# jianfch/stable-ts

Measured on AMD Instinct MI355X. Metric: real-time factor (audio-sec/wall-sec) large-v3 word_timestamps=True, higher is better.
Workload: dtype f16; 1 GPU; large-v3 (random-init, weight recipe BENCH_WEIGHTS = the parity-pinned recipe of tests/test_gpu_f16_depth.py), 10 min synthetic 16 kHz audio per GPU, word_timestamps=True, beam_size=5, 112 decode steps/window, window-parallel batch 20, default regrouping inside the timed pass; mode=transcribe, windows_per_gpu=20, segments=125, words=1670, parallelism=dp1 (windows sharded, no data-path collective)

## Files before the change

### include/swx.h

```cpp
#ifndef SWX_H
#define SWX_H
#include <stdint.h>
#include <stddef.h>

#ifdef __cplusplus
extern "C" {
#endif

#define SWX_F32 0
#define SWX_F16 1

#define SWX_N_SAMPLES 480000
#define SWX_N_FRAMES 3000
#define SWX_N_FFT 400
#define SWX_HOP 160

typedef struct swx_dims {
    int32_t n_mels, n_audio_ctx, n_audio_state, n_audio_head, n_audio_layer;
    int32_t n_vocab, n_text_ctx, n_text_state, n_text_head, n_text_layer;
} swx_dims;

typedef struct swx_model swx_model;

const char *swx_strerror(int code);
// ... 99 lines not shown
int swx_pcm_edit(const float *d_clean, float *d_probe, int64_t stride, int n_rows, const int32_t *d_ops,
                 const int32_t *d_row_start, int n_ops, void *stream);

typedef struct swx_flac_info {
    int32_t sample_rate, channels, bits_per_sample, min_block, max_block;
    int64_t total_samples;
    uint8_t md5[16];
} swx_flac_info;
int swx_flac_probe(const uint8_t *h_data, size_t n_bytes, swx_flac_info *info);
int64_t swx_flac_decode(const uint8_t *h_data, size_t n_bytes, int32_t *h_out, int64_t capacity_frames, swx_flac_info *info);

size_t swx_dtw_workspace_bytes(int W, int ld_n, int ld_m);
int swx_dtw(const float *d_x, int W, int ld_n, int ld_m, const int32_t *d_N, const int32_t *d_M,
            int32_t *d_text_idx, int32_t *d_time_idx, int32_t *d_len, void *d_trace_ws, void *stream);

int swx_prof_enable(int on);
int swx_debug_flags(int flags);
int swx_prof_collect(double *out, int n_classes);
int swx_graph_stats(const swx_model *m, int64_t *out);

int swx_test_gemm(int dtype, const void *d_a, int64_t lda, const void *d_w, const float *d_bias, const void *d_res,
                  void *d_c, int64_t ldc, int M, int N, int K, int epilogue, int force_kernel, void *stream);
int swx_test_gemm_plan(int M, int N, int K, int epilogue, int force_kernel, int flags);
int swx_test_dec_gemm(const void *d_a, int64_t lda, const void *d_w, const float *d_gamma, const float *d_beta,
                      const float *d_bias, void *d_c, int64_t ldc, void *d_x, void *d_kcache, void *d_vcache,
                      const int32_t *d_pos0, int n_ctx, int d, int M, int N, int K, int epilogue, void *d_scratch,
                      size_t scratch_bytes, void *stream);
int swx_test_layernorm(int dtype, const void *d_x, const float *d_g, const float *d_b, void *d_y, int rows, int d,
                       void *stream);
int swx_test_attention(int dtype, const void *d_q, int64_t ldq, const void *d_k, const void *d_v, int64_t ldkv,
                       void *d_o, int64_t ldo, int B, int H, int nq, int nk, int force_kernel, int vt_kp, void *stream);

int swx_test_self_attn_step(const void *d_q, void *d_kcache, void *d_vcache, const int32_t *d_anc, const int32_t *d_pos0,
                            int R, int H, int n_ctx, int d, int variant, void *d_o, void *stream);

int swx_test_self_attn_multi(const void *d_q, void *d_kcache, void *d_vcache, int R, int H, int n_new, int n_ctx, int d, int mq,
                             void *d_o, void *stream);

int swx_test_self_attn_general(int dtype, const void *d_qkv, int64_t ldqkv, void *d_kcache, void *d_vcache, const int32_t *d_anc,
                               const int32_t *d_pos0, int R, int H, int n_new, int n_ctx, int d, int row_mul, int skip_append,
                               int pos0_all_zero, void *d_o, void *stream);
int swx_test_kcache_index(int k_chunked, int n_ctx, int d, int pos, int h, int chunk);
int swx_test_kcache_relayout(const void *h_src, void *h_dst, int64_t rows, int n_ctx, int d, int elem_bytes, int to_chunked);
int swx_test_dec_gemm_kl(const void *d_a, int64_t lda, const void *d_w, const float *d_gamma, const float *d_beta,
                         const float *d_bias, void *d_c, int64_t ldc, void *d_x, void *d_kcache, void *d_vcache,
                         const int32_t *d_pos0, int n_ctx, int d, int M, int N, int K, int epilogue, int rps, int k_chunked,
// ... 30 lines not shown
```

### stable_ts_amd/_lib.py

```python
import ctypes
import os
from ctypes import POINTER, Structure, c_char_p, c_float, c_int, c_int32, c_int64, c_size_t, c_uint64, c_void_p

_HERE = os.path.dirname(os.path.abspath(__file__))
LIB_PATH = os.path.join(_HERE, "libswx.so")

SWX_F32 = 0
SWX_F16 = 1


class SwxError(RuntimeError):
    pass


class swx_dims(Structure):
    _fields_ = [(n, c_int32) for n in ("n_mels", "n_audio_ctx", "n_audio_state", "n_audio_head", "n_audio_layer",
                                       "n_vocab", "n_text_ctx", "n_text_state", "n_text_head", "n_text_layer")]


class swx_flac_info(Structure):
    _fields_ = [("sample_rate", c_int32), ("channels", c_int32), ("bits_per_sample", c_int32), ("min_block", c_int32),
                ("max_block", c_int32), ("total_samples", c_int64), ("md5", ctypes.c_uint8 * 16)]


# ... 54 lines not shown
                                       c_void_p, c_void_p, c_void_p, c_void_p]),
    "swx_test_next_token_reduce": (c_int, [c_void_p, c_int64, c_int, c_int, c_void_p, c_int, c_void_p, c_void_p, c_void_p,
                                           c_void_p]),
    "swx_detect_language": (c_int, [c_void_p, c_void_p, c_int, c_int, c_void_p, c_int, c_void_p, c_void_p, c_void_p]),
    "swx_align_weights_scratch_bytes":(c_size_t, [c_int, c_int, c_int]),
    "swx_align_weights": (c_int, [c_void_p, c_int, c_int, c_int, c_int, POINTER(c_int32), c_float, c_int, c_void_p,
                                  c_void_p, c_size_t, c_void_p]),
    "swx_median_filter": (c_int, [c_void_p, c_int64, c_int, c_int, c_void_p, c_void_p]),
    "swx_loudness_probe": (c_int, [c_void_p, c_int64, c_void_p, c_void_p, c_int, c_int, c_void_p, c_void_p, c_size_t, c_void_p]),
    "swx_loudness_probe_scratch_bytes": (c_size_t, [c_int]),
    "swx_pcm_edit": (c_int, [c_void_p, c_void_p, c_int64, c_int, c_void_p, c_void_p, c_int, c_void_p]),
    "swx_flac_probe": (c_int, [c_void_p, c_size_t, POINTER(swx_flac_info)]),
    "swx_flac_decode": (c_int64, [c_void_p, c_size_t, c_void_p, c_int64, POINTER(swx_flac_info)]),
    "swx_dtw_workspace_bytes": (c_size_t, [c_int, c_int, c_int]),
    "swx_dtw": (c_int, [c_void_p, c_int, c_int, c_int, c_void_p, c_void_p, c_void_p, c_void_p, c_void_p, c_void_p,
                        c_void_p]),
    "swx_prof_enable": (c_int, [c_int]),
    "swx_debug_flags": (c_int, [c_int]),
    "swx_prof_collect": (c_int, [POINTER(ctypes.c_double), c_int]),
    "swx_graph_stats": (c_int, [c_void_p, POINTER(c_int64)]),
    "swx_test_gemm": (c_int, [c_int, c_void_p, c_int64, c_void_p, c_void_p, c_void_p, c_void_p, c_int64, c_int, c_int,
                              c_int, c_int, c_int, c_void_p]),
    "swx_test_gemm_plan": (c_int, [c_int, c_int, c_int, c_int, c_int, c_int]),
    "swx_test_dec_gemm": (c_int, [c_void_p, c_int64, c_void_p, c_void_p, c_void_p, c_void_p, c_void_p, c_int64, c_void_p,
                                  c_void_p, c_void_p, c_void_p, c_int, c_int, c_int, c_int, c_int, c_int, c_void_p, c_size_t,
                                  c_void_p]),
    "swx_test_self_attn_step": (c_int, [c_void_p, c_void_p, c_void_p, c_void_p, c_void_p, c_int, c_int, c_int, c_int, c_int, c_void_p,
                                        c_void_p]),
    "swx_test_self_attn_multi": (c_int, [c_void_p, c_void_p, c_void_p, c_int, c_int, c_int, c_int, c_int, c_int, c_void_p, c_void_p]),
    "swx_test_self_attn_general": (c_int, [c_int, c_void_p, c_int64, c_void_p, c_void_p, c_void_p, c_void_p, c_int, c_int, c_int, c_int,
                                           c_int, c_int, c_int, c_int, c_void_p, c_void_p]),
    "swx_test_kcache_index": (c_int, [c_int] * 6),
    "swx_test_kcache_relayout": (c_int, [c_void_p, c_void_p, c_int64, c_int, c_int, c_int, c_int]),
    "swx_test_dec_gemm_kl": (c_int, [c_void_p, c_int64, c_void_p, c_void_p, c_void_p, c_void_p, c_void_p, c_int64, c_void_p,
                                     c_void_p, c_void_p, c_void_p, c_int, c_int, c_int, c_int, c_int, c_int, c_int, c_int, c_void_p,
                                     c_size_t, c_void_p]),
    "swx_test_self_attn_step_kl": (c_int, [c_void_p, c_void_p, c_void_p, c_void_p, c_void_p, c_int, c_int, c_int, c_int, c_int, c_int,
                                           c_void_p, c_void_p]),
    "swx_test_self_attn_multi_kl": (c_int, [c_void_p, c_void_p, c_void_p, c_int, c_int, c_int, c_int, c_int, c_int, c_int, c_void_p,
                                            c_void_p]),
    "swx_test_self_attn_general_kl": (c_int, [c_int, c_void_p, c_int64, c_void_p, c_void_p, c_void_p, c_void_p, c_int, c_int, c_int,
                                              c_int, c_int, c_int, c_int, c_int, c_int, c_int, c_void_p, c_void_p]),
    "swx_test_self_attn_plan": (c_int, [c_int] * 12),
    "swx_test_dec_plan": (c_int, [c_int, c_int, c_int, c_int, c_int]),
    "swx_test_gelu_pair": (c_int, [c_void_p, c_void_p]),
    "swx_test_decode_script_ws_bytes": (c_size_t, [POINTER(swx_decode_cfg), c_int, c_int]),
# ... 44 lines not shown
```

### stable_ts_amd/csrc/swx_gemm.hip

```cpp
#include <cstdlib>
#include <type_traits>
#include <array>
#include <vector>
#include <cstdio>
#include "swx_common.h"
#include "swx_kernels.h"

namespace {

template <typename T>
__device__ __forceinline__ void epilogue_store(const GemmArgs &g, int row, int col, float v)
{
    if (row >= g.M || col >= g.N) return;
    if (g.epi & EPI_BIAS) v += g.bias[col];
    if (g.epi & EPI_GELU) v = gelu_erf(v);
    if (g.epi & EPI_RESF32MOD) v += g.Rf[(size_t)(row % g.res_mod) * g.N + col];
    if (g.epi & EPI_RES) v += to_f32<T>(((const T *)g.R)[(size_t)row * g.ldr + col]);
    if (g.epi & EPI_STORE_VT) {
        const int w = row / g.vt_s, sidx = row - w * g.vt_s;
        ((T *)g.C)[(size_t)w * g.vt_bs + (size_t)col * g.vt_kp + sidx] = from_f32<T>(v);
    } else if (g.epi & EPI_CBATCH) {
        const int w = row / g.vt_s, sidx = row - w * g.vt_s;
        ((T *)g.C)[(size_t)w * g.vt_bs + (size_t)sidx * g.ldc + col] = from_f32<T>(v);
    } else if (g.epi & EPI_OUT_F32) ((float *)g.C)[(size_t)row * g.ldc + col] = v;
// ... 967 lines not shown
    if (K % 32 != 0) return -4;
    const bool skinny_ok = M <= 128 && K % 128 == 0 && K / 128 <= 10 && N <= 16384;
    if (force_kernel == 2) return skinny_ok ? SWX_GEMM_SKINNY : -4;
    if (skinny_ok && force_kernel != 1 && force_kernel < 7) return SWX_GEMM_SKINNY;
    const bool glds_ok = K % 64 == 0 && ptr16;
    if (force_kernel >= 7 && !glds_ok) return -4;
    if (force_kernel == 1 || !glds_ok) return SWX_GEMM_TILED_REG;
    const int64_t t128 = (int64_t)cdiv(N, BN) * cdiv(M, BM);
    const bool narrow = force_kernel == 8 || (force_kernel != 9 && N % 64 == 0 && t128 < 224);
    const bool big_ok = !(epi & ~(EPI_BIAS | EPI_GELU | EPI_RES)) && ldc % 8 == 0 && (!(epi & EPI_RES) || ldr % 8 == 0);
    if (force_kernel == 12) return big_ok && K >= 128 ? SWX_GEMM_BIG : -4;
    const int64_t t256 = (int64_t)cdiv(M, BG) * cdiv(N, BG);
    const double fill = (double)t256 / (double)(((t256 + 255) / 256) * 256);
    if (force_kernel == 0 && big_ok && t256 >= 200 && K >= 512 && (fill >= 0.9 || (fill >= 0.75 && K >= 2560)) &&
        !(flags & SWX_FLAG_NO_BIG_TILE))
        return SWX_GEMM_BIG;
    const bool ring_ok = K >= 128;
    if (force_kernel == 10 || force_kernel == 11) return !ring_ok ? -4 : force_kernel == 10 ? SWX_GEMM_RING64 : SWX_GEMM_RING128;
    if (force_kernel == 0 && ring_ok && M > 256 && (narrow || t128 <= 256) && !(flags & SWX_FLAG_NO_RING))
        return narrow ? SWX_GEMM_RING64 : SWX_GEMM_RING128;
    return narrow ? SWX_GEMM_GLDS64 : SWX_GEMM_GLDS128;
}

int swx_gemm(int dtype, const GemmArgs &g, int force_kernel, hipStream_t s)
{
    if (g.M <= 0 || g.N <= 0) return 0;
    if (dtype == SWX_F16) {
        if (g.lda % 8 != 0 || g.ldw % 8 != 0) return -4;
        const bool ptr16 = (uintptr_t)g.A % 16 == 0 && (uintptr_t)g.W % 16 == 0;
        const bool cr16 = (uintptr_t)g.C % 16 == 0 && (!(g.epi & EPI_RES) || (uintptr_t)g.R % 16 == 0);
        const int plan = swx_gemm_plan_f16(g.M, g.N, g.K, g.epi, cr16 ? g.ldc : 1, cr16 ? g.ldr : 1, ptr16, force_kernel, swx_flags());
        if (plan < 0) return plan;
        if (plan == SWX_GEMM_SKINNY) {
            SwxProfScope prof(PC_GEMM_SKINNY, 2.0 * ((double)g.N * g.K + (double)g.M * g.K) + (double)g.M * g.N * ((g.epi & EPI_OUT_F32) ? 4 : 2), s);
            dim3 grid(cdiv(g.N, 16));
            const int mt = cdiv(g.M, 16);
            switch (mt) {
                case 1: hipLaunchKernelGGL(gemm_f16_skinny<1>, grid, dim3(256), 0, s, g); break;
                case 2: hipLaunchKernelGGL(gemm_f16_skinny<2>, grid, dim3(256), 0, s, g); break;
                case 3: hipLaunchKernelGGL(gemm_f16_skinny<3>, grid, dim3(256), 0, s, g); break;
                case 4: hipLaunchKernelGGL(gemm_f16_skinny<4>, grid, dim3(256), 0, s, g); break;
                case 5: hipLaunchKernelGGL(gemm_f16_skinny<5>, grid, dim3(256), 0, s, g); break;
                case 6: hipLaunchKernelGGL(gemm_f16_skinny<6>, grid, dim3(256), 0, s, g); break;
                case 7: hipLaunchKernelGGL(gemm_f16_skinny<7>, grid, dim3(256), 0, s, g); break;
                default: hipLaunchKernelGGL(gemm_f16_skinny<8>, grid, dim3(256), 0, s, g); break;
            }
        } else {
            SwxProfScope prof(PC_GEMM_TILED, 2.0 * (double)g.M * g.N * g.K, s);
            const dim3 grid(cdiv(g.N, BN), cdiv(g.M, BM));
            switch (plan) {
                case SWX_GEMM_BIG: {
                    GemmArgs gb = g;
                    gb.tile_order = (swx_flags() & SWX_FLAG_BIG8_GROUPED) ? 1 : 0;
                    hipLaunchKernelGGL(gemm_f16_big8, dim3(cdiv(g.N, BG), cdiv(g.M, BG)), dim3(512), 2 * B8_BUF, s, gb); break;
// ... 25 lines not shown
```

### stable_ts_amd/csrc/swx_kernels.h

```cpp
#pragma once
#include <hip/hip_runtime.h>
#include <stdint.h>
#include "../../include/swx.h"

#define EPI_BIAS 1
#define EPI_GELU 2
#define EPI_RES 4
#define EPI_OUT_F32 8
#define EPI_RESF32MOD 16
#define EPI_CBATCH 64
#define EPI_STORE_VT 32
#define EPI_KV 128

#define EPI_QKV_VT 256

struct GemmArgs {
    const void *A; int64_t lda;
    const void *W; int64_t ldw;
    const float *bias;
    const void *R; int64_t ldr;
    const float *Rf; int res_mod;
    void *C; int64_t ldc;
    void *C2;
    void *P; int64_t p_bs;
    int p_nkpad, p_vcol0;
    int M, N, K;
    int epi;
    int vt_s, vt_kp; int64_t vt_bs;
    int vt_zero_pad;
    int tile_order;
};
int swx_gemm(int dtype, const GemmArgs &g, int force_kernel, hipStream_t s);
enum { SWX_GEMM_TILED_REG = 0, SWX_GEMM_SKINNY = 1, SWX_GEMM_GLDS128 = 2, SWX_GEMM_GLDS64 = 3, SWX_GEMM_RING64 = 4, SWX_GEMM_RING128 = 5,
       SWX_GEMM_BIG = 6 };
int swx_gemm_plan_f16(int M, int N, int K, int epi, int64_t ldc, int64_t ldr, bool ptr16, int force_kernel, int flags);

#define SWX_FLAG_NO_FAST_STEP 1
#define SWX_FLAG_NO_PACKED_XKV 2048
#define SWX_FLAG_SELECT_MEM 8192
#define SWX_FLAG_NO_GRAPH 16384
#define SWX_FLAG_NO_PREFETCH 32768
#define SWX_FLAG_NO_RING 65536
#define SWX_FLAG_SCORE_TILED 262144
#define SWX_FLAG_NO_TALL 524288
#define SWX_FLAG_NO_FUSED_XQ 1048576
#define SWX_FLAG_TICKET 2097152
#define SWX_FLAG_BIG8_GROUPED 4194304
#define SWX_FLAG_XKV_TWO_LAUNCHES 8388608
#define SWX_FLAG_LOUDNESS_ONE_WG 16777216
#define SWX_FLAG_XATTN_R5 33554432
#define SWX_FLAG_FLASH_PIPELINED 67108864
#define SWX_FLAG_SELFATTN_WG5 134217728
#define SWX_FLAG_QKV_SEPARATE_VT 268435456
#define SWX_FLAG_SELFATTN_NO_DEEP 4
#define SWX_FLAG_DEC_NO_W1 16
#define SWX_FLAG_TALL_NO_W8 32
#define SWX_FLAG_SELFATTN_NO_MQ 256
#define SWX_FLAG_FLASH_NO_QB1 64
#define SWX_FLAG_XKV_PACK_SEPARATE 128
#define SWX_FLAG_DEC_W1_FULL_TILE 256
#define SWX_FLAG_XQ_FULL_TILE 512
#define SWX_FLAG_KCACHE_CHUNKED 2
#define SWX_FLAG_NO_BIG_TILE 131072
#define SWX_DEFAULT_FLAGS 0
int swx_flags();

struct KLayout { int sp, sh, sc; };
__host__ __device__ inline KLayout swx_klayout(int chunked, int n_ctx, int d)
{
    return chunked ? KLayout{8, 64 * n_ctx, 8 * n_ctx} : KLayout{d, 64, 8};
}
__host__ __device__ inline int swx_kidx(const KLayout &L, int pos, int h, int chunk) { return h * L.sh + chunk * L.sc + pos * L.sp; }

#define DEC_LN 1
#define DEC_GELU 2
#define DEC_RES 4
#define DEC_QKV 8
#define DEC_SLAB 16
#define DEC_TICKET 32
struct DecPrefetch {
    const void *base;
    int lines;
};
DecPrefetch swx_dec_prefetch_of(const void *packed_w, int M, int N, int K, int epi);

struct DecGemmArgs {
    const _Float16 *A; int64_t lda;
    const _Float16 *W; int64_t ldw;
// ... 124 lines not shown
```

### stable_ts_amd/csrc/swx_runtime.hip

```cpp
#include <algorithm>
#include <map>
#include <memory>
#include <string>
#include <vector>
#include <cmath>
#include <cstring>
#include <cstdio>
#include <cstdlib>
#include "swx_common.h"
#include "swx_kernels.h"
#include "swx_decode.h"

namespace {

enum SlotKind { SK_MAT = 0, SK_VEC = 1, SK_CONV = 2 };

struct Slot {
    size_t off = 0;
    int kind = SK_VEC;
    int64_t rows = 0, cols = 0;
    int64_t dst_ld = 0;
    bool loaded = false;
};

// ... 36 lines not shown
        size_t tokens0, tokens1, anc0, anc1, pos0, win_begin, sum_lp, sum_lp_next, row_done, win_done, win_done_prev, n_done;
        size_t fin_tokens, fin_score, fin_len, fin_count, cand_lp, cand_tok, logits, hid2;
        size_t kcache, vcache, sk, sv, cap, mean, sd, suppress, slabs, heads, win_uid;
        size_t total;
        int64_t rows_big, logits_rows;
        size_t slab_bytes;
    } L;

    template <typename P> P *A(size_t off) const { return (P *)(arena + off); }
    template <typename P> P *Wp(size_t off) const { return (P *)(ws + off); }

    struct StepGraph { std::vector<uint64_t> key; hipGraph_t graph = nullptr; hipGraphExec_t exec = nullptr; uint64_t used = 0; };
    std::vector<StepGraph> graphs;
    uint64_t graph_clock = 0;
    std::vector<int32_t> ragged_hv;
    hipStream_t cap_stream = nullptr;
    bool graphs_off = false;
    int graph_failures = 0;
    int64_t n_captures = 0, n_replays = 0, n_eager_units = 0;
    void drop_graphs() {
        for (auto &g : graphs) { if (g.exec) (void)hipGraphExecDestroy(g.exec); if (g.graph) (void)hipGraphDestroy(g.graph); }
        graphs.clear();
    }
    ~swx_model() { drop_graphs(); if (cap_stream) (void)hipStreamDestroy(cap_stream); }
};

namespace {

constexpr int FIN_CAP = 32;
constexpr int MAX_GROUP = 16;
constexpr int MAX_SUPPRESS = 4096;
constexpr int SMALL_I32 = 8192;

size_t add_slot(swx_model *m, size_t &cur, const std::string &name, int kind, int64_t rows, int64_t cols, int64_t dst_ld,
                size_t bytes, size_t base_off = (size_t)-1, size_t sub_off = 0)
{
    Slot s;
    s.kind = kind; s.rows = rows; s.cols = cols; s.dst_ld = dst_ld;
    if (base_off == (size_t)-1) { s.off = cur; cur = align_up(cur + bytes); }
    else s.off = base_off + sub_off;
    m->slots[name] = s;
    return s.off;
}

void build_layout(swx_model *m)
{
    const swx_dims &D = m->dims;
// ... 177 lines not shown

hipEvent_t prof_event()
{
    if (g_pool_next == g_pool.size()) {
        hipEvent_t e;
        if (hipEventCreate(&e) != hipSuccess) return nullptr;
        g_pool.push_back(e);
    }
    return g_pool[g_pool_next++];
}

#define SWX_TRY(expr) do { int _r = (expr); if (_r < 0) return _r; } while (0)

GemmArgs gemm_args(const void *A, int64_t lda, const void *W, int64_t ldw, const float *bias, void *C, int64_t ldc,
                   int M, int N, int K, int epi)
{
    GemmArgs g{};
    g.A = A; g.lda = lda; g.W = W; g.ldw = ldw; g.bias = bias; g.C = C; g.ldc = ldc; g.M = M; g.N = N; g.K = K; g.epi = epi;
    g.R = nullptr; g.ldr = 0; g.Rf = nullptr; g.res_mod = 1;
    return g;
}

int gemm_residual(swx_model *m, const void *A, int64_t lda, size_t w_off, size_t b_off, void *X, int64_t ldx, int M, int N,
                  int K, hipStream_t s)
{
    GemmArgs g = gemm_args(A, lda, m->arena + w_off, K, m->A<float>(b_off), X, ldx, M, N, K, EPI_BIAS | EPI_RES);
    g.R = X; g.ldr = ldx;
    return swx_gemm(m->dtype, g, 0, s);
}

inline int64_t xkv_plain_elems(const swx_dims &D)
{
    return (int64_t)D.n_audio_ctx * D.n_text_state + (int64_t)D.n_text_state * SWX_VT_KP;
}
inline int64_t xkv_packed_elems(const swx_dims &D)
{
    return (int64_t)D.n_text_head * swx_xkv_packed_elems_per_head(D.n_audio_ctx);
}
inline int64_t xkv_chunk_elems(const swx_model *m)
{
    return xkv_plain_elems(m->dims) + (m->dtype == SWX_F16 ? xkv_packed_elems(m->dims) : 0);
}

struct FwdCfg {
    int W;
    int rpw;
    int row_mul;
    int n_new;
    const int32_t *tokens; int64_t ld_tok;
    int xkv_W;
    const int32_t *pos0;
    unsigned char *kcache, *vcache;
// ... 464 lines not shown
    __syncthreads();
    mx = fmaxf(fmaxf(red[0], red[1]), fmaxf(red[2], red[3]));
    __syncthreads();
    float sum = 0.f;
    for (int j = tid; j < n_lang; j += 256) {
        const float x = lg[j];
        if (x == mx) atomicMin(&best_j, j);
        const float p = expf(x - mx);
        lg[j] = p;
        sum += p;
    }
    sum = wave_sum(sum);
    if (lane == 0) red[wave] = sum;
    __syncthreads();
    sum = (red[0] + red[1]) + (red[2] + red[3]);
    for (int j = tid; j < n_lang; j += 256) probs[(size_t)w * n_lang + j] = lg[j] / sum;
    if (tid == 0) best[w] = best_j < n_lang ? lang_tokens[best_j] : -1;
}

}

bool swx_prof_on() { return g_prof_enabled; }
int swx_flags() { return g_debug_flags; }
void swx_prof_begin(int cls, double work, hipStream_t s)
{
    ProfRec r{cls, work, prof_event(), prof_event()};
    if (!r.a || !r.b) return;
    (void)hipEventRecord(r.a, s);
    g_prof.push_back(r);
}
void swx_prof_end(hipStream_t s)
{
    if (!g_prof.empty()) (void)hipEventRecord(g_prof.back().b, s);
}

__global__ __launch_bounds__(64) void lane_xor_check_kernel(const uint32_t *__restrict__ in, uint32_t *__restrict__ out)
{
    const int lane = threadIdx.x;
    const uint32_t x = in[blockIdx.x * 64 + lane];
    uint32_t *o = out + (size_t)blockIdx.x * 13 * 64 + lane;
    o[0 * 64] = lane_xor_u32<32>(x, lane); o[1 * 64] = lane_xor_u32<16>(x, lane); o[2 * 64] = lane_xor_u32<8>(x, lane);
    o[3 * 64] = lane_xor_u32<4>(x, lane);  o[4 * 64] = lane_xor_u32<2>(x, lane);  o[5 * 64] = lane_xor_u32<1>(x, lane);
    o[6 * 64] = (uint32_t)__shfl_xor((int)x, 32, 64); o[7 * 64] = (uint32_t)__shfl_xor((int)x, 16, 64);
    o[8 * 64] = (uint32_t)__shfl_xor((int)x, 8, 64);  o[9 * 64] = (uint32_t)__shfl_xor((int)x, 4, 64);
    o[10 * 64] = (uint32_t)__shfl_xor((int)x, 2, 64); o[11 * 64] = (uint32_t)__shfl_xor((int)x, 1, 64);
    double v = (double)__uint_as_float(x);
// ... 282 lines not shown
    std::vector<int32_t> lens((size_t)B * 2);
    for (int b = 0; b < B; ++b) {
        if (n_total[b] <= 200 || n_total[b] / 160 > 3008 || n_valid[b] < 0 || n_valid[b] > n_total[b] ||
            n_valid[b] > 480000)
            return -2;
        lens[2 * b] = n_valid[b];
        lens[2 * b + 1] = n_total[b];
    }
    hipStream_t s = S(stream);
    int32_t *d_lens = m->Wp<int32_t>(m->L.h1);
    hipError_t e = hipMemcpyAsync(d_lens, lens.data(), lens.size() * 4, hipMemcpyHostToDevice, s);
    if (e == hipSuccess) e = hipStreamSynchronize(s);
    if (e != hipSuccess) return -100 - (int)e;
    return swx_mel_ragged_launch(d_pcm, d_lens, B, m->A<float>(m->o_hann), m->A<double2>(m->o_twiddle),
                                 m->A<float>(m->o_filters), m->dims.n_mels, d_mel, m->Wp<unsigned>(m->L.gmax), group, s);
}

int swx_log_mel_ragged(swx_model *m, const float *d_pcm, const int32_t *n_valid, const int32_t *n_total, int B,
                       float *d_mel, int per_item_max, void *stream)
{
    return swx_log_mel_ragged_grouped(m, d_pcm, n_valid, n_total, B, d_mel, per_item_max ? 1 : B, stream);
}

int swx_encode(swx_model *m, const float *d_mel, int B, void *d_xa, void *stream)
{
    if (!m || !m->arena || !m->ws) return -9;
    if (B <= 0) return 0;
    if (B > m->max_windows) return -8;
    const swx_dims &D = m->dims;
    const int d = D.n_audio_state, H = D.n_audio_head, S_ = D.n_audio_ctx;
    const size_t e = m->esz;
    hipStream_t s = S(stream);
    unsigned char *melT = m->ws + m->L.melT, *h1 = m->ws + m->L.h1;
    unsigned char *x = m->ws + m->L.x, *h = m->ws + m->L.h, *qkv = m->ws + m->L.qkv, *att = m->ws + m->L.att, *u = m->ws + m->L.u;
    const int rows = B * S_;
    if (D.n_audio_ctx != 1500) return -2;

    SWX_TRY(swx_mel_transpose(m->dtype, d_mel, B, D.n_mels, m->Cp, melT, s));
    SWX_TRY(swx_fill_zero(h1, (size_t)B * 3002 * d * e, s));
    for (int b = 0; b < B; ++b) {
        const unsigned char *a = melT + (size_t)b * 3002 * m->Cp * e;
        unsigned char *c = h1 + ((size_t)b * 3002 + 1) * d * e;
        SWX_TRY(swx_gemm(m->dtype, gemm_args(a, m->Cp, m->arena + m->o_conv1_w, 3 * m->Cp, m->A<float>(m->o_conv1_b), c, d,
                                             3000, d, 3 * m->Cp, EPI_BIAS | EPI_GELU), 0, s));
    }
    for (int b = 0; b < B; ++b) {
        const unsigned char *a = h1 + (size_t)b * 3002 * d * e;
        GemmArgs g = gemm_args(a, 2 * d, m->arena + m->o_conv2_w, 3 * d, m->A<float>(m->o_conv2_b), x + (size_t)b * S_ * d * e, d,
                               S_, d, 3 * d, EPI_BIAS | EPI_GELU | EPI_RESF32MOD);
        g.Rf = m->A<float>(m->o_enc_pos); g.res_mod = S_;
        SWX_TRY(swx_gemm(m->dtype, g, 0, s));
    }
    for (int l = 0; l < D.n_audio_layer; ++l) {
        const LayerW &w = m->enc[l];
        SWX_TRY(swx_layernorm(m->dtype, x, d, m->A<float>(w.ln1_g), m->A<float>(w.ln1_b), h, d, rows, d, s));
        const bool fuse_vt = m->dtype == SWX_F16 && d % 128 == 0 && S_ % 4 == 0 && !(g_debug_flags & SWX_FLAG_QKV_SEPARATE_VT) &&
                             swx_gemm_plan_f16(rows, 3 * d, d, EPI_BIAS, 3 * d, 1, true, 0, g_debug_flags) != SWX_GEMM_BIG;
        {
            GemmArgs gq = gemm_args(h, d, m->arena + w.wqkv, d, m->A<float>(w.bqkv), qkv, 3 * d, rows, 3 * d, d, EPI_BIAS | (fuse_vt ? EPI_QKV_VT : 0));
            if (fuse_vt) { gq.C2 = u; gq.vt_s = S_; gq.vt_kp = SWX_VT_KP; gq.vt_bs = (int64_t)H * 64 * SWX_VT_KP; gq.vt_zero_pad = 1; }
            SWX_TRY(swx_gemm(m->dtype, gq, 0, s));
        }
        AttnArgs a{};
        a.q = qkv; a.ldq = 3 * d; a.k = qkv + (size_t)d * e; a.v = qkv + (size_t)2 * d * e; a.ldkv = 3 * d; a.o = att; a.ldo = d;
        a.k_bs = (int64_t)S_ * 3 * d; a.v_bs = a.k_bs; a.vt_kp = 0;
        a.B = B; a.H = H; a.nq = S_; a.nk = S_; a.q_rows_per_batch = S_;
        if (m->dtype == SWX_F16) {
            if (!fuse_vt) SWX_TRY(swx_transpose_v(a.v, 3 * d, a.v_bs, S_, u, SWX_VT_KP, (int64_t)H * 64 * SWX_VT_KP, B, H, s));
            a.v = u; a.vt_kp = SWX_VT_KP; a.v_bs = (int64_t)H * 64 * SWX_VT_KP;
        }
        SWX_TRY(swx_attention(m->dtype, a, 0, s));
        SWX_TRY(gemm_residual(m, att, d, w.wo, w.bo, x, d, rows, d, d, s));
        SWX_TRY(swx_layernorm(m->dtype, x, d, m->A<float>(w.ln2_g), m->A<float>(w.ln2_b), h, d, rows, d, s));
        SWX_TRY(swx_gemm(m->dtype, gemm_args(h, d, m->arena + w.w1, d, m->A<float>(w.b1), u, 4 * d, rows, 4 * d, d, EPI_BIAS | EPI_GELU), 0, s));
        SWX_TRY(gemm_residual(m, u, 4 * d, w.w2, w.b2, x, d, rows, d, 4 * d, s));
    }
    SWX_TRY(swx_layernorm(m->dtype, x, d, m->A<float>(m->o_lnpost_g), m->A<float>(m->o_lnpost_b), d_xa, d, rows, d, s));
    return 0;
}

size_t swx_cross_kv_bytes(const swx_model *m, int B)
{
    if (!m) return 0;
    return (size_t)m->dims.n_text_layer * B * (size_t)xkv_chunk_elems(m) * m->esz;
}

int swx_cross_kv(swx_model *m, const void *d_xa, int B, void *d_xkv, void *stream)
{
    if (!m || !m->arena) return -9;
    const swx_dims &D = m->dims;
    const int d = D.n_text_state, S_ = D.n_audio_ctx;
    const size_t e = m->esz;
    if (D.n_audio_state != d) return -1;
    const int64_t chunk = xkv_chunk_elems(m);
    hipStream_t s = S(stream);
    SWX_TRY(swx_pad_zero((unsigned char *)d_xkv + (size_t)S_ * d * e, (int64_t)SWX_VT_KP * e, chunk * (int64_t)e, (int)(S_ * e),
                         (int)((SWX_VT_KP - S_) * e), d, D.n_text_layer * B, s));
    for (int l = 0; l < D.n_text_layer; ++l) {
        const LayerW &w = m->dec[l];
        unsigned char *base = (unsigned char *)d_xkv + (size_t)l * B * chunk * e;
        const bool one_launch = m->dtype == SWX_F16 && d % 128 == 0 && (int64_t)B * S_ > 128 && !(g_debug_flags & SWX_FLAG_XKV_TWO_LAUNCHES);
        bool packed_by_epilogue = false;
        if (one_launch) {
            GemmArgs gkv = gemm_args(d_xa, d, m->arena + w.wckv, d, m->A<float>(w.bckv), base, d, B * S_, 2 * d, d, EPI_BIAS | EPI_KV);
            gkv.vt_s = S_; gkv.vt_kp = SWX_VT_KP; gkv.vt_bs = chunk; gkv.C2 = base + (size_t)S_ * d * e;
            if (!(g_debug_flags & SWX_FLAG_XKV_PACK_SEPARATE)) {
                gkv.P = base + (size_t)xkv_plain_elems(D) * e; gkv.p_bs = chunk; gkv.p_nkpad = ((S_ + 31) / 32) * 32; gkv.p_vcol0 = d;
                packed_by_epilogue = true;
            }
            SWX_TRY(swx_gemm(m->dtype, gkv, 0, s));
        } else {
        GemmArgs gk = gemm_args(d_xa, d, m->arena + w.wckv, d, m->A<float>(w.bckv), base, d, B * S_, d, d, EPI_BIAS | EPI_CBATCH);
        gk.vt_s = S_; gk.vt_kp = 0; gk.vt_bs = chunk;
        SWX_TRY(swx_gemm(m->dtype, gk, 0, s));
        GemmArgs gv = gemm_args(d_xa, d, m->arena + w.wckv + (size_t)d * d * e, d, m->A<float>(w.bckv) + d,
                                base + (size_t)S_ * d * e, d, B * S_, d, d, EPI_BIAS | EPI_STORE_VT);
        gv.vt_s = S_; gv.vt_kp = SWX_VT_KP; gv.vt_bs = chunk;
        SWX_TRY(swx_gemm(m->dtype, gv, 0, s));
        }
        if (m->dtype == SWX_F16 && !packed_by_epilogue)
            SWX_TRY(swx_xkv_pack(base, base + (size_t)S_ * d * e, base + (size_t)xkv_plain_elems(D) * e, B, D.n_text_head, S_, d,
                                 SWX_VT_KP, chunk, s));
    }
    return 0;
}

namespace {
__global__ __launch_bounds__(64) void gather_rows_kernel(const unsigned char *__restrict__ src, const int32_t *__restrict__ idx,
                                                         unsigned char *__restrict__ dst, int row_bytes)
{
    const int j = blockIdx.x;
    const uint4 *sp = (const uint4 *)(src + (size_t)idx[j] * row_bytes);
    uint4 *dp = (uint4 *)(dst + (size_t)j * row_bytes);
    for (int i = threadIdx.x; i < row_bytes / 16; i += 64) dp[i] = sp[i];
}

constexpr int DECODE_POLL = 8;
int decode_loop_stop(int i, int n_min, int n_ctx, int min_tokens, int sample_len, int W, const int32_t *d_n_done, hipStream_t s)
{
    const int steps = i + 1;
    if (n_min + i + 1 > n_ctx) return 1;
    if ((steps % DECODE_POLL == 0 && steps >= min_tokens) || steps == sample_len) {
        int32_t h_done = 0;
        hipError_t er = hipMemcpyAsync(&h_done, d_n_done, 4, hipMemcpyDeviceToHost, s);
        if (er != hipSuccess) return -100 - (int)er;
        er = hipStreamSynchronize(s);
        if (er != hipSuccess) return -100 - (int)er;
// ... 535 lines not shown
{
    if (W <= 0) return 0;
    if (!d_scratch || scratch_bytes < swx_align_weights_scratch_bytes(W, H, N)) return -8;
    hipStream_t s = S(stream);
    float *rstat = (float *)d_scratch;
    int32_t *cnt = (int32_t *)((unsigned char *)d_scratch + align_up((size_t)W * H * N * sizeof(float2)));
    std::vector<int32_t> hv(2 * W);
    for (int w = 0; w < W; ++w) { hv[w] = N; hv[W + w] = h_n_frames[w]; }
    hipError_t er = hipMemcpyAsync(cnt, hv.data(), hv.size() * 4, hipMemcpyHostToDevice, s);
    if (er == hipSuccess) er = hipStreamSynchronize(s);
    if (er != hipSuccess) return -100 - (int)er;
    return swx_align_weights_launch(d_qk, rstat, nullptr, nullptr, W, H, N, ld_f, cnt, cnt + W, qk_scale, medfilt_width, d_neg_matrix,
                                    N, ld_f, s);
}

int swx_test_gemm(int dtype, const void *d_a, int64_t lda, const void *d_w, const float *d_bias, const void *d_res,
                  void *d_c, int64_t ldc, int M, int N, int K, int epilogue, int force_kernel, void *stream)
{
    GemmArgs g = gemm_args(d_a, lda, d_w, K, d_bias, d_c, ldc, M, N, K, epilogue);
    g.R = d_res; g.ldr = ldc;
    return swx_gemm(dtype, g, force_kernel, S(stream));
}

int swx_test_gemm_plan(int M, int N, int K, int epilogue, int force_kernel, int flags)
{
    return swx_gemm_plan_f16(M, N, K, epilogue, N, N, true, force_kernel, flags);
}

int swx_test_dec_gemm(const void *d_a, int64_t lda, const void *d_w, const float *d_gamma, const float *d_beta, const float *d_bias,
                      void *d_c, int64_t ldc, void *d_x, void *d_kcache, void *d_vcache, const int32_t *d_pos0, int n_ctx, int d,
                      int M, int N, int K, int epilogue, void *d_scratch, size_t scratch_bytes, void *stream)
{
    return swx_test_dec_gemm_kl(d_a, lda, d_w, d_gamma, d_beta, d_bias, d_c, ldc, d_x, d_kcache, d_vcache, d_pos0, n_ctx, d, M, N, K, epilogue,
                                0, 0, d_scratch, scratch_bytes, stream);
}

int swx_test_dec_gemm_kl(const void *d_a, int64_t lda, const void *d_w, const float *d_gamma, const float *d_beta, const float *d_bias,
                         void *d_c, int64_t ldc, void *d_x, void *d_kcache, void *d_vcache, const int32_t *d_pos0, int n_ctx, int d,
                         int M, int N, int K, int epilogue, int rps, int k_chunked, void *d_scratch, size_t scratch_bytes, void *stream)
{
    if (k_chunked && (epilogue & DEC_QKV) && (n_ctx <= 0 || d <= 0 || d % 64)) return -2;
    hipStream_t s = S(stream);
    unsigned char *p = (unsigned char *)d_scratch;
    const size_t slab_b = align_up(swx_dec_slab_floats(M, N, K) * 4 + 256);
    const size_t need = align_up((size_t)N * K * 2) + 2 * align_up((size_t)N * 4) + slab_b + (size_t)SWX_DEC_TICKETS * 4;
    if (scratch_bytes < need) return -8;
// ... 319 lines not shown
```

Baseline: 1438 x real time.

## Split encoder and cross-KV batches across two streams for concurrent execution

The encoder batch is split into two halves that are enqueued on the main stream and a side stream, joined with events, so their kernels can overlap on the GPU. Cross-attention KV projection layers alternate between the two streams in the same way. GEMM tile planning keeps using the full-batch row count so the kernel choice does not change. The cost is an extra stream and events, plus smaller per-launch GEMMs that may use the GPU less efficiently than one large batched launch.

```diff
diff --git a/include/swx.h b/include/swx.h
--- a/include/swx.h
+++ b/include/swx.h
@@ -145,6 +145,8 @@
 int swx_test_gemm(int dtype, const void *d_a, int64_t lda, const void *d_w, const float *d_bias, const void *d_res,
                   void *d_c, int64_t ldc, int M, int N, int K, int epilogue, int force_kernel, void *stream);
 int swx_test_gemm_plan(int M, int N, int K, int epilogue, int force_kernel, int flags);
+int swx_test_encode_groups(int B, int split_min, int32_t *out);
+int swx_test_set_encode_split_min(swx_model *m, int n);
 int swx_test_dec_gemm(const void *d_a, int64_t lda, const void *d_w, const float *d_gamma, const float *d_beta,
                       const float *d_bias, void *d_c, int64_t ldc, void *d_x, void *d_kcache, void *d_vcache,
                       const int32_t *d_pos0, int n_ctx, int d, int M, int N, int K, int epilogue, void *d_scratch,
diff --git a/stable_ts_amd/_lib.py b/stable_ts_amd/_lib.py
--- a/stable_ts_amd/_lib.py
+++ b/stable_ts_amd/_lib.py
@@ -100,6 +100,8 @@
     "swx_test_gemm": (c_int, [c_int, c_void_p, c_int64, c_void_p, c_void_p, c_void_p, c_void_p, c_int64, c_int, c_int,
                               c_int, c_int, c_int, c_void_p]),
     "swx_test_gemm_plan": (c_int, [c_int, c_int, c_int, c_int, c_int, c_int]),
+    "swx_test_encode_groups": (c_int, [c_int, c_int, POINTER(c_int32)]),
+    "swx_test_set_encode_split_min": (c_int, [c_void_p, c_int]),
     "swx_test_dec_gemm": (c_int, [c_void_p, c_int64, c_void_p, c_void_p, c_void_p, c_void_p, c_void_p, c_int64, c_void_p,
                                   c_void_p, c_void_p, c_void_p, c_int, c_int, c_int, c_int, c_int, c_int, c_void_p, c_size_t,
                                   c_void_p]),
diff --git a/stable_ts_amd/csrc/swx_gemm.hip b/stable_ts_amd/csrc/swx_gemm.hip
--- a/stable_ts_amd/csrc/swx_gemm.hip
+++ b/stable_ts_amd/csrc/swx_gemm.hip
@@ -1013,14 +1013,14 @@
     return narrow ? SWX_GEMM_GLDS64 : SWX_GEMM_GLDS128;
 }
 
-int swx_gemm(int dtype, const GemmArgs &g, int force_kernel, hipStream_t s)
+int swx_gemm(int dtype, const GemmArgs &g, int force_kernel, hipStream_t s, int plan_rows)
 {
     if (g.M <= 0 || g.N <= 0) return 0;
     if (dtype == SWX_F16) {
         if (g.lda % 8 != 0 || g.ldw % 8 != 0) return -4;
         const bool ptr16 = (uintptr_t)g.A % 16 == 0 && (uintptr_t)g.W % 16 == 0;
         const bool cr16 = (uintptr_t)g.C % 16 == 0 && (!(g.epi & EPI_RES) || (uintptr_t)g.R % 16 == 0);
-        const int plan = swx_gemm_plan_f16(g.M, g.N, g.K, g.epi, cr16 ? g.ldc : 1, cr16 ? g.ldr : 1, ptr16, force_kernel, swx_flags());
+        const int plan = swx_gemm_plan_f16(plan_rows > g.M ? plan_rows : g.M, g.N, g.K, g.epi, cr16 ? g.ldc : 1, cr16 ? g.ldr : 1, ptr16, force_kernel, swx_flags());
         if (plan < 0) return plan;
         if (plan == SWX_GEMM_SKINNY) {
             SwxProfScope prof(PC_GEMM_SKINNY, 2.0 * ((double)g.N * g.K + (double)g.M * g.K) + (double)g.M * g.N * ((g.epi & EPI_OUT_F32) ? 4 : 2), s);
diff --git a/stable_ts_amd/csrc/swx_kernels.h b/stable_ts_amd/csrc/swx_kernels.h
--- a/stable_ts_amd/csrc/swx_kernels.h
+++ b/stable_ts_amd/csrc/swx_kernels.h
@@ -30,7 +30,7 @@
     int vt_zero_pad;
     int tile_order;
 };
-int swx_gemm(int dtype, const GemmArgs &g, int force_kernel, hipStream_t s);
+int swx_gemm(int dtype, const GemmArgs &g, int force_kernel, hipStream_t s, int plan_rows = 0);
 enum { SWX_GEMM_TILED_REG = 0, SWX_GEMM_SKINNY = 1, SWX_GEMM_GLDS128 = 2, SWX_GEMM_GLDS64 = 3, SWX_GEMM_RING64 = 4, SWX_GEMM_RING128 = 5,
        SWX_GEMM_BIG = 6 };
 int swx_gemm_plan_f16(int M, int N, int K, int epi, int64_t ldc, int64_t ldr, bool ptr16, int force_kernel, int flags);
@@ -61,9 +61,13 @@
 #define SWX_FLAG_DEC_W1_FULL_TILE 256
 #define SWX_FLAG_XQ_FULL_TILE 512
 #define SWX_FLAG_KCACHE_CHUNKED 2
+#define SWX_FLAG_ENC_ONE_STREAM 4096
 #define SWX_FLAG_NO_BIG_TILE 131072
 #define SWX_DEFAULT_FLAGS 0
 int swx_flags();
+
+#define SWX_ENCODE_SPLIT_MIN 8
+int swx_encode_groups(int B, int split_min, int32_t out[4]);
 
 struct KLayout { int sp, sh, sc; };
 __host__ __device__ inline KLayout swx_klayout(int chunked, int n_ctx, int d)
diff --git a/stable_ts_amd/csrc/swx_runtime.hip b/stable_ts_amd/csrc/swx_runtime.hip
--- a/stable_ts_amd/csrc/swx_runtime.hip
+++ b/stable_ts_amd/csrc/swx_runtime.hip
@@ -82,7 +82,16 @@
         for (auto &g : graphs) { if (g.exec) (void)hipGraphExecDestroy(g.exec); if (g.graph) (void)hipGraphDestroy(g.graph); }
         graphs.clear();
     }
-    ~swx_model() { drop_graphs(); if (cap_stream) (void)hipStreamDestroy(cap_stream); }
+    hipStream_t side_stream = nullptr;
+    hipEvent_t ev_fork = nullptr, ev_join = nullptr;
+    int encode_split_min = SWX_ENCODE_SPLIT_MIN;
+    ~swx_model() {
+        drop_graphs();
+        if (cap_stream) (void)hipStreamDestroy(cap_stream);
+        if (side_stream) (void)hipStreamDestroy(side_stream);
+        if (ev_fork) (void)hipEventDestroy(ev_fork);
+        if (ev_join) (void)hipEventDestroy(ev_join);
+    }
 };
 
 namespace {
@@ -306,12 +315,32 @@
 }
 
 int gemm_residual(swx_model *m, const void *A, int64_t lda, size_t w_off, size_t b_off, void *X, int64_t ldx, int M, int N,
-                  int K, hipStream_t s)
+                  int K, hipStream_t s, int plan_rows = 0)
 {
     GemmArgs g = gemm_args(A, lda, m->arena + w_off, K, m->A<float>(b_off), X, ldx, M, N, K, EPI_BIAS | EPI_RES);
     g.R = X; g.ldr = ldx;
-    return swx_gemm(m->dtype, g, 0, s);
-}
+    return swx_gemm(m->dtype, g, 0, s, plan_rows);
+}
+
+int enc_fork(swx_model *m, hipStream_t s)
+{
+    if (!m->side_stream && hipStreamCreateWithFlags(&m->side_stream, hipStreamNonBlocking) != hipSuccess) { m->side_stream = nullptr; return -3; }
+    if (!m->ev_fork && hipEventCreateWithFlags(&m->ev_fork, hipEventDisableTiming) != hipSuccess) { m->ev_fork = nullptr; return -3; }
+    if (!m->ev_join && hipEventCreateWithFlags(&m->ev_join, hipEventDisableTiming) != hipSuccess) { m->ev_join = nullptr; return -3; }
+    hipError_t e = hipEventRecord(m->ev_fork, s);
+    if (e == hipSuccess) e = hipStreamWaitEvent(m->side_stream, m->ev_fork, 0);
+    return e == hipSuccess ? 0 : -100 - (int)e;
+}
+
+int enc_join(swx_model *m, hipStream_t s)
+{
+    hipError_t e = hipEventRecord(m->ev_join, m->side_stream);
+    if (e == hipSuccess) e = hipStreamWaitEvent(s, m->ev_join, 0);
+    if (e != hipSuccess) { (void)hipStreamSynchronize(m->side_stream); return -100 - (int)e; }
+    return 0;
+}
+
+bool enc_two_streams() { return !g_prof_enabled && !(g_debug_flags & SWX_FLAG_ENC_ONE_STREAM); }
 
 inline int64_t xkv_plain_elems(const swx_dims &D)
 {
@@ -822,6 +851,15 @@
 
 bool swx_prof_on() { return g_prof_enabled; }
 int swx_flags() { return g_debug_flags; }
+
+int swx_encode_groups(int B, int split_min, int32_t out[4])
+{
+    out[0] = 0; out[1] = B > 0 ? B : 0; out[2] = out[1]; out[3] = 0;
+    if (B <= 0) return 0;
+    if (B < 2 || B < split_min) return 1;
+    out[1] = (B + 1) / 2; out[2] = out[1]; out[3] = B / 2;
+    return 2;
+}
 void swx_prof_begin(int cls, double work, hipStream_t s)
 {
     ProfRec r{cls, work, prof_event(), prof_event()};
@@ -1150,67 +1188,164 @@
     return swx_log_mel_ragged_grouped(m, d_pcm, n_valid, n_total, B, d_mel, per_item_max ? 1 : B, stream);
 }
 
+namespace {
+struct EncGroup {
+    swx_model *m; hipStream_t s; int b0, nb;
+    int plan_rows;
+    const float *mel;
+    unsigned char *melT, *h1, *x, *h, *qkv, *att, *u, *xa;
+
+    EncGroup(swx_model *m_, hipStream_t s_, int b0_, int nb_, int B, const float *d_mel, void *d_xa) : m(m_), s(s_), b0(b0_), nb(nb_)
+    {
+        const swx_dims &D = m->dims;
+        const size_t e = m->esz, d = D.n_audio_state, row0 = (size_t)b0 * D.n_audio_ctx;
+        plan_rows = B * D.n_audio_ctx;
+        mel = d_mel + (size_t)b0 * D.n_mels * 3000;
+        melT = m->ws + m->L.melT + (size_t)b0 * 3002 * m->Cp * e;
+        h1 = m->ws + m->L.h1 + (size_t)b0 * 3002 * d * e;
+        x = m->ws + m->L.x + row0 * d * e;
+        h = m->ws + m->L.h + row0 * d * e;
+        qkv = m->ws + m->L.qkv + row0 * 3 * d * e;
+        att = m->ws + m->L.att + row0 * d * e;
+        u = m->ws + m->L.u + row0 * 4 * d * e;
+        xa = (unsigned char *)d_xa + row0 * d * e;
+    }
+
+    int stem_begin() const
+    {
+        SWX_TRY(swx_mel_transpose(m->dtype, mel, nb, m->dims.n_mels, m->Cp, melT, s));
+        return swx_fill_zero(h1, (size_t)nb * 3002 * m->dims.n_audio_state * m->esz, s);
+    }
+    int conv1(int b) const
+    {
+        const int d = m->dims.n_audio_state;
+        const size_t e = m->esz;
+        const unsigned char *a = melT + (size_t)b * 3002 * m->Cp * e;
+        unsigned char *c = h1 + ((size_t)b * 3002 + 1) * d * e;
+        return swx_gemm(m->dtype, gemm_args(a, m->Cp, m->arena + m->o_conv1_w, 3 * m->Cp, m->A<float>(m->o_conv1_b), c, d,
+                                            3000, d, 3 * m->Cp, EPI_BIAS | EPI_GELU), 0, s);
+    }
+    int conv2(int b) const
+    {
+        const int d = m->dims.n_audio_state, S_ = m->dims.n_audio_ctx;
+        const size_t e = m->esz;
+        const unsigned char *a = h1 + (size_t)b * 3002 * d * e;
+        GemmArgs g = gemm_args(a, 2 * d, m->arena + m->o_conv2_w, 3 * d, m->A<float>(m->o_conv2_b), x + (size_t)b * S_ * d * e, d,
+                               S_, d, 3 * d, EPI_BIAS | EPI_GELU | EPI_RESF32MOD);
+        g.Rf = m->A<float>(m->o_enc_pos); g.res_mod = S_;
+        return swx_gemm(m->dtype, g, 0, s);
+    }
+    int layer(int l) const
+    {
+        const swx_dims &D = m->dims;
+        const int d = D.n_audio_state, H = D.n_audio_head, S_ = D.n_audio_ctx, rows = nb * S_;
+        const size_t e = m->esz;
+        const LayerW &w = m->enc[l];
+        SWX_TRY(swx_layernorm(m->dtype, x, d, m->A<float>(w.ln1_g), m->A<float>(w.ln1_b), h, d, rows, d, s));
+        const bool fuse_vt = m->dtype == SWX_F16 && d % 128 == 0 && S_ % 4 == 0 && !(g_debug_flags & SWX_FLAG_QKV_SEPARATE_VT) &&
+                             swx_gemm_plan_f16(plan_rows, 3 * d, d, EPI_BIAS, 3 * d, 1, true, 0, g_debug_flags) != SWX_GEMM_BIG;
+        {
+            GemmArgs gq = gemm_args(h, d, m->arena + w.wqkv, d, m->A<float>(w.bqkv), qkv, 3 * d, rows, 3 * d, d, EPI_BIAS | (fuse_vt ? EPI_QKV_VT : 0));
+            if (fuse_vt) { gq.C2 = u; gq.vt_s = S_; gq.vt_kp = SWX_VT_KP; gq.vt_bs = (int64_t)H * 64 * SWX_VT_KP; gq.vt_zero_pad = 1; }
+            SWX_TRY(swx_gemm(m->dtype, gq, 0, s, plan_rows));
+        }
+        AttnArgs a{};
+        a.q = qkv; a.ldq = 3 * d; a.k = qkv + (size_t)d * e; a.v = qkv + (size_t)2 * d * e; a.ldkv = 3 * d; a.o = att; a.ldo = d;
+        a.k_bs = (int64_t)S_ * 3 * d; a.v_bs = a.k_bs; a.vt_kp = 0;
+        a.B = nb; a.H = H; a.nq = S_; a.nk = S_; a.q_rows_per_batch = S_;
+        if (m->dtype == SWX_F16) {
+            if (!fuse_vt) SWX_TRY(swx_transpose_v(a.v, 3 * d, a.v_bs, S_, u, SWX_VT_KP, (int64_t)H * 64 * SWX_VT_KP, nb, H, s));
+            a.v = u; a.vt_kp = SWX_VT_KP; a.v_bs = (int64_t)H * 64 * SWX_VT_KP;
+        }
+        SWX_TRY(swx_attention(m->dtype, a, 0, s));
+        SWX_TRY(gemm_residual(m, att, d, w.wo, w.bo, x, d, rows, d, d, s, plan_rows));
+        SWX_TRY(swx_layernorm(m->dtype, x, d, m->A<float>(w.ln2_g), m->A<float>(w.ln2_b), h, d, rows, d, s));
+        SWX_TRY(swx_gemm(m->dtype, gemm_args(h, d, m->arena + w.w1, d, m->A<float>(w.b1), u, 4 * d, rows, 4 * d, d, EPI_BIAS | EPI_GELU), 0, s, plan_rows));
+        return gemm_residual(m, u, 4 * d, w.w2, w.b2, x, d, rows, d, 4 * d, s, plan_rows);
+    }
+    int ln_post() const
+    {
+        const int d = m->dims.n_audio_state;
+        return swx_layernorm(m->dtype, x, d, m->A<float>(m->o_lnpost_g), m->A<float>(m->o_lnpost_b), xa, d, nb * m->dims.n_audio_ctx, d, s);
+    }
+};
+
+int encode_enqueue(const EncGroup *g, int ng, int n_layer)
+{
+    int nb_max = 0;
+    for (int i = 0; i < ng; ++i) { SWX_TRY(g[i].stem_begin()); nb_max = g[i].nb > nb_max ? g[i].nb : nb_max; }
+    for (int b = 0; b < nb_max; ++b)
+        for (int i = 0; i < ng; ++i) if (b < g[i].nb) SWX_TRY(g[i].conv1(b));
+    for (int b = 0; b < nb_max; ++b)
+        for (int i = 0; i < ng; ++i) if (b < g[i].nb) SWX_TRY(g[i].conv2(b));
+    for (int l = 0; l < n_layer; ++l)
+        for (int i = 0; i < ng; ++i) SWX_TRY(g[i].layer(l));
+    for (int i = 0; i < ng; ++i) SWX_TRY(g[i].ln_post());
+    return 0;
+}
+}
+
 int swx_encode(swx_model *m, const float *d_mel, int B, void *d_xa, void *stream)
 {
     if (!m || !m->arena || !m->ws) return -9;
     if (B <= 0) return 0;
     if (B > m->max_windows) return -8;
     const swx_dims &D = m->dims;
-    const int d = D.n_audio_state, H = D.n_audio_head, S_ = D.n_audio_ctx;
-    const size_t e = m->esz;
     hipStream_t s = S(stream);
-    unsigned char *melT = m->ws + m->L.melT, *h1 = m->ws + m->L.h1;
-    unsigned char *x = m->ws + m->L.x, *h = m->ws + m->L.h, *qkv = m->ws + m->L.qkv, *att = m->ws + m->L.att, *u = m->ws + m->L.u;
-    const int rows = B * S_;
     if (D.n_audio_ctx != 1500) return -2;
 
-    SWX_TRY(swx_mel_transpose(m->dtype, d_mel, B, D.n_mels, m->Cp, melT, s));
-    SWX_TRY(swx_fill_zero(h1, (size_t)B * 3002 * d * e, s));
-    for (int b = 0; b < B; ++b) {
-        const unsigned char *a = melT + (size_t)b * 3002 * m->Cp * e;
-        unsigned char *c = h1 + ((size_t)b * 3002 + 1) * d * e;
-        SWX_TRY(swx_gemm(m->dtype, gemm_args(a, m->Cp, m->arena + m->o_conv1_w, 3 * m->Cp, m->A<float>(m->o_conv1_b), c, d,
-                                             3000, d, 3 * m->Cp, EPI_BIAS | EPI_GELU), 0, s));
-    }
-    for (int b = 0; b < B; ++b) {
-        const unsigned char *a = h1 + (size_t)b * 3002 * d * e;
-        GemmArgs g = gemm_args(a, 2 * d, m->arena + m->o_conv2_w, 3 * d, m->A<float>(m->o_conv2_b), x + (size_t)b * S_ * d * e, d,
-                               S_, d, 3 * d, EPI_BIAS | EPI_GELU | EPI_RESF32MOD);
-        g.Rf = m->A<float>(m->o_enc_pos); g.res_mod = S_;
-        SWX_TRY(swx_gemm(m->dtype, g, 0, s));
-    }
-    for (int l = 0; l < D.n_audio_layer; ++l) {
-        const LayerW &w = m->enc[l];
-        SWX_TRY(swx_layernorm(m->dtype, x, d, m->A<float>(w.ln1_g), m->A<float>(w.ln1_b), h, d, rows, d, s));
-        const bool fuse_vt = m->dtype == SWX_F16 && d % 128 == 0 && S_ % 4 == 0 && !(g_debug_flags & SWX_FLAG_QKV_SEPARATE_VT) &&
-                             swx_gemm_plan_f16(rows, 3 * d, d, EPI_BIAS, 3 * d, 1, true, 0, g_debug_flags) != SWX_GEMM_BIG;
-        {
-            GemmArgs gq = gemm_args(h, d, m->arena + w.wqkv, d, m->A<float>(w.bqkv), qkv, 3 * d, rows, 3 * d, d, EPI_BIAS | (fuse_vt ? EPI_QKV_VT : 0));
-            if (fuse_vt) { gq.C2 = u; gq.vt_s = S_; gq.vt_kp = SWX_VT_KP; gq.vt_bs = (int64_t)H * 64 * SWX_VT_KP; gq.vt_zero_pad = 1; }
-            SWX_TRY(swx_gemm(m->dtype, gq, 0, s));
-        }
-        AttnArgs a{};
-        a.q = qkv; a.ldq = 3 * d; a.k = qkv + (size_t)d * e; a.v = qkv + (size_t)2 * d * e; a.ldkv = 3 * d; a.o = att; a.ldo = d;
-        a.k_bs = (int64_t)S_ * 3 * d; a.v_bs = a.k_bs; a.vt_kp = 0;
-        a.B = B; a.H = H; a.nq = S_; a.nk = S_; a.q_rows_per_batch = S_;
-        if (m->dtype == SWX_F16) {
-            if (!fuse_vt) SWX_TRY(swx_transpose_v(a.v, 3 * d, a.v_bs, S_, u, SWX_VT_KP, (int64_t)H * 64 * SWX_VT_KP, B, H, s));
-            a.v = u; a.vt_kp = SWX_VT_KP; a.v_bs = (int64_t)H * 64 * SWX_VT_KP;
-        }
-        SWX_TRY(swx_attention(m->dtype, a, 0, s));
-        SWX_TRY(gemm_residual(m, att, d, w.wo, w.bo, x, d, rows, d, d, s));
-        SWX_TRY(swx_layernorm(m->dtype, x, d, m->A<float>(w.ln2_g), m->A<float>(w.ln2_b), h, d, rows, d, s));
-        SWX_TRY(swx_gemm(m->dtype, gemm_args(h, d, m->arena + w.w1, d, m->A<float>(w.b1), u, 4 * d, rows, 4 * d, d, EPI_BIAS | EPI_GELU), 0, s));
-        SWX_TRY(gemm_residual(m, u, 4 * d, w.w2, w.b2, x, d, rows, d, 4 * d, s));
-    }
-    SWX_TRY(swx_layernorm(m->dtype, x, d, m->A<float>(m->o_lnpost_g), m->A<float>(m->o_lnpost_b), d_xa, d, rows, d, s));
-    return 0;
+    int32_t grp[4];
+    const int ng = swx_encode_groups(B, enc_two_streams() ? m->encode_split_min : B + 1, grp);
+    if (ng == 1) {
+        const EncGroup g(m, s, 0, B, B, d_mel, d_xa);
+        return encode_enqueue(&g, 1, D.n_audio_layer);
+    }
+    SWX_TRY(enc_fork(m, s));
+    const EncGroup g[2] = { EncGroup(m, s, grp[0], grp[1], B, d_mel, d_xa), EncGroup(m, m->side_stream, grp[2], grp[3], B, d_mel, d_xa) };
+    const int rc = encode_enqueue(g, 2, D.n_audio_layer);
+    const int rj = enc_join(m, s);
+    return rc < 0 ? rc : rj;
 }
 
 size_t swx_cross_kv_bytes(const swx_model *m, int B)
 {
     if (!m) return 0;
     return (size_t)m->dims.n_text_layer * B * (size_t)xkv_chunk_elems(m) * m->esz;
+}
+
+namespace {
+int cross_kv_layer(swx_model *m, const void *d_xa, int B, void *d_xkv, int l, hipStream_t s)
+{
+    const swx_dims &D = m->dims;
+    const int d = D.n_text_state, S_ = D.n_audio_ctx;
+    const size_t e = m->esz;
+    const int64_t chunk = xkv_chunk_elems(m);
+    const LayerW &w = m->dec[l];
+    unsigned char *base = (unsigned char *)d_xkv + (size_t)l * B * chunk * e;
+    const bool one_launch = m->dtype == SWX_F16 && d % 128 == 0 && (int64_t)B * S_ > 128 && !(g_debug_flags & SWX_FLAG_XKV_TWO_LAUNCHES);
+    bool packed_by_epilogue = false;
+    if (one_launch) {
+        GemmArgs gkv = gemm_args(d_xa, d, m->arena + w.wckv, d, m->A<float>(w.bckv), base, d, B * S_, 2 * d, d, EPI_BIAS | EPI_KV);
+        gkv.vt_s = S_; gkv.vt_kp = SWX_VT_KP; gkv.vt_bs = chunk; gkv.C2 = base + (size_t)S_ * d * e;
+        if (!(g_debug_flags & SWX_FLAG_XKV_PACK_SEPARATE)) {
+            gkv.P = base + (size_t)xkv_plain_elems(D) * e; gkv.p_bs = chunk; gkv.p_nkpad = ((S_ + 31) / 32) * 32; gkv.p_vcol0 = d;
+            packed_by_epilogue = true;
+        }
+        SWX_TRY(swx_gemm(m->dtype, gkv, 0, s));
+    } else {
+    GemmArgs gk = gemm_args(d_xa, d, m->arena + w.wckv, d, m->A<float>(w.bckv), base, d, B * S_, d, d, EPI_BIAS | EPI_CBATCH);
+    gk.vt_s = S_; gk.vt_kp = 0; gk.vt_bs = chunk;
+    SWX_TRY(swx_gemm(m->dtype, gk, 0, s));
+    GemmArgs gv = gemm_args(d_xa, d, m->arena + w.wckv + (size_t)d * d * e, d, m->A<float>(w.bckv) + d,
+                            base + (size_t)S_ * d * e, d, B * S_, d, d, EPI_BIAS | EPI_STORE_VT);
+    gv.vt_s = S_; gv.vt_kp = SWX_VT_KP; gv.vt_bs = chunk;
+    SWX_TRY(swx_gemm(m->dtype, gv, 0, s));
+    }
+    if (m->dtype == SWX_F16 && !packed_by_epilogue)
+        SWX_TRY(swx_xkv_pack(base, base + (size_t)S_ * d * e, base + (size_t)xkv_plain_elems(D) * e, B, D.n_text_head, S_, d,
+                             SWX_VT_KP, chunk, s));
+    return 0;
+}
 }
 
 int swx_cross_kv(swx_model *m, const void *d_xa, int B, void *d_xkv, void *stream)
@@ -1224,33 +1359,13 @@
     hipStream_t s = S(stream);
     SWX_TRY(swx_pad_zero((unsigned char *)d_xkv + (size_t)S_ * d * e, (int64_t)SWX_VT_KP * e, chunk * (int64_t)e, (int)(S_ * e),
                          (int)((SWX_VT_KP - S_) * e), d, D.n_text_layer * B, s));
-    for (int l = 0; l < D.n_text_layer; ++l) {
-        const LayerW &w = m->dec[l];
-        unsigned char *base = (unsigned char *)d_xkv + (size_t)l * B * chunk * e;
-        const bool one_launch = m->dtype == SWX_F16 && d % 128 == 0 && (int64_t)B * S_ > 128 && !(g_debug_flags & SWX_FLAG_XKV_TWO_LAUNCHES);
-        bool packed_by_epilogue = false;
-        if (one_launch) {
-            GemmArgs gkv = gemm_args(d_xa, d, m->arena + w.wckv, d, m->A<float>(w.bckv), base, d, B * S_, 2 * d, d, EPI_BIAS | EPI_KV);
-            gkv.vt_s = S_; gkv.vt_kp = SWX_VT_KP; gkv.vt_bs = chunk; gkv.C2 = base + (size_t)S_ * d * e;
-            if (!(g_debug_flags & SWX_FLAG_XKV_PACK_SEPARATE)) {
-                gkv.P = base + (size_t)xkv_plain_elems(D) * e; gkv.p_bs = chunk; gkv.p_nkpad = ((S_ + 31) / 32) * 32; gkv.p_vcol0 = d;
-                packed_by_epilogue = true;
-            }
-            SWX_TRY(swx_gemm(m->dtype, gkv, 0, s));
-        } else {
-        GemmArgs gk = gemm_args(d_xa, d, m->arena + w.wckv, d, m->A<float>(w.bckv), base, d, B * S_, d, d, EPI_BIAS | EPI_CBATCH);
-        gk.vt_s = S_; gk.vt_kp = 0; gk.vt_bs = chunk;
-        SWX_TRY(swx_gemm(m->dtype, gk, 0, s));
-        GemmArgs gv = gemm_args(d_xa, d, m->arena + w.wckv + (size_t)d * d * e, d, m->A<float>(w.bckv) + d,
-                                base + (size_t)S_ * d * e, d, B * S_, d, d, EPI_BIAS | EPI_STORE_VT);
-        gv.vt_s = S_; gv.vt_kp = SWX_VT_KP; gv.vt_bs = chunk;
-        SWX_TRY(swx_gemm(m->dtype, gv, 0, s));
-        }
-        if (m->dtype == SWX_F16 && !packed_by_epilogue)
-            SWX_TRY(swx_xkv_pack(base, base + (size_t)S_ * d * e, base + (size_t)xkv_plain_elems(D) * e, B, D.n_text_head, S_, d,
-                                 SWX_VT_KP, chunk, s));
-    }
-    return 0;
+    int32_t grp[4];
+    const bool two = D.n_text_layer >= 2 && swx_encode_groups(B, enc_two_streams() ? m->encode_split_min : B + 1, grp) == 2;
+    if (two) SWX_TRY(enc_fork(m, s));
+    int rc = 0;
+    for (int l = 0; l < D.n_text_layer && rc >= 0; ++l) rc = cross_kv_layer(m, d_xa, B, d_xkv, l, two && (l & 1) ? m->side_stream : s);
+    if (two) { const int rj = enc_join(m, s); if (rc >= 0) rc = rj; }
+    return rc < 0 ? rc : 0;
 }
 
 namespace {
@@ -1832,6 +1947,16 @@
     return swx_gemm(dtype, g, force_kernel, S(stream));
 }
 
+int swx_test_encode_groups(int B, int split_min, int32_t *out) { return out ? swx_encode_groups(B, split_min, out) : -1; }
+
+int swx_test_set_encode_split_min(swx_model *m, int n)
+{
+    if (!m) return -1;
+    const int old = m->encode_split_min;
+    m->encode_split_min = n > 0 ? n : SWX_ENCODE_SPLIT_MIN;
+    return old;
+}
+
 int swx_test_gemm_plan(int M, int N, int K, int epilogue, int force_kernel, int flags)
 {
     return swx_gemm_plan_f16(M, N, K, epilogue, N, N, true, force_kernel, flags);
```

Measured after the change: 1438 x real time (median of 2 runs). No clear change (+0.0%).
